# simonsysu/tfs

Measured on AMD Instinct MI355X. Metric: GiB/s CRC32 verify, device-resident 64 KiB files; 1/2/4/8 MI355X, higher is better.
Workload: dtype u8

## Files before the change

tfs_amd/csrc/crc_math.h:

```cpp
#pragma once
#include <cstdint>

namespace tfscrc {

constexpr uint32_t kPoly = 0xEDB88320u;

inline void make_byte_table(uint32_t t[256]) {
  for (uint32_t i = 0; i < 256; ++i) {
    uint32_t c = i;
    for (int k = 0; k < 8; ++k) c = (c & 1u) ? (c >> 1) ^ kPoly : (c >> 1);
    t[i] = c;
  }
}

inline void make_slice_tables(uint32_t s[][256], int nslices) {
  make_byte_table(s[0]);
  for (int k = 1; k < nslices; ++k)
    for (int b = 0; b < 256; ++b) s[k][b] = (s[k - 1][b] >> 8) ^ s[0][s[k - 1][b] & 0xffu];
}

inline uint32_t multmodp(uint32_t a, uint32_t b) {
  uint32_t m = 1u << 31, p = 0;
  for (;;) {
    if (a & m) {
      p ^= b;
      if ((a & (m - 1)) == 0) break;
    }
    m >>= 1;
    b = (b & 1u) ? (b >> 1) ^ kPoly : b >> 1;
  }
  return p;
}

inline uint32_t x2nmodp(uint64_t n, unsigned k) {
  uint32_t p = 1u << 31;
  uint32_t sq = 1u << 30;
  for (unsigned i = 0; i < k; ++i) sq = multmodp(sq, sq);
  while (n) {
    if (n & 1) p = multmodp(sq, p);
    n >>= 1;
    sq = multmodp(sq, sq);
  }
  return p;
}

inline uint32_t shift_bytes(uint32_t c, uint64_t nbytes) { return multmodp(x2nmodp(nbytes, 3), c); }

inline uint32_t shift_bytes_pow(uint32_t c, uint64_t nbytes) {
  struct Pow {
    uint32_t p[64];
    Pow() {
      p[0] = x2nmodp(1, 3);
      for (int k = 1; k < 64; ++k) p[k] = multmodp(p[k - 1], p[k - 1]);
    }
  };
  static const Pow pw;
  for (int k = 0; nbytes; ++k, nbytes >>= 1)
    if (nbytes & 1) c = multmodp(pw.p[k], c);
  return c;
}

inline void make_shift_table(uint32_t t[4][256], uint64_t nbytes) {
  const uint32_t k = x2nmodp(nbytes, 3);
  for (int j = 0; j < 4; ++j)
    for (uint32_t b = 0; b < 256; ++b) t[j][b] = multmodp(k, b << (8 * j));
}

inline void make_shift_table5(uint32_t t[7][32], uint64_t nbytes) {
  const uint32_t k = x2nmodp(nbytes, 3);
  for (int j = 0; j < 7; ++j)
    for (uint32_t e = 0; e < 32; ++e) t[j][e] = (j == 6 && e >= 4) ? 0u : multmodp(k, e << (5 * j));
}

}
```

tfs_amd/csrc/tfs_ec_abi.cpp:

```cpp
#include <hip/hip_runtime.h>

#include <cstdlib>
#include <cstring>
#include <mutex>
#include <vector>

#include "../../include/tfs_ec.h"
#include "crc_math.h"
#include "ec_math.h"

#include "ec_locate_plan.h"
#include "ec_marshal_plan.h"
#include "ec_read_plan.h"
#include "tfs_ec_device.h"

extern "C" int tfs_crc32_dev_malloc(tfs_crc_ctx* ctx, uint64_t bytes, void** d_ptr);
extern "C" int tfs_crc32_dev_free(tfs_crc_ctx* ctx, void* d_ptr);
extern "C" void* tfs_crc32_stream(tfs_crc_ctx* ctx);

using namespace tfsec;

namespace {
struct Plan {
  std::vector<int> sources, outputs;
// ... 172 lines not shown
int upload_read_tables(tfs_ec* ec) {
  void* d = nullptr;
  const int rc = tfs_crc32_dev_malloc(ec->ctx, sizeof(ReadTables), &d);
  if (rc) return rc;
  if (hipMemcpy(d, &read_tables(), sizeof(ReadTables), hipMemcpyHostToDevice) != hipSuccess) {
    tfs_crc32_dev_free(ec->ctx, d);
    return TFS_CRC_EXIT_DEVICE_ERROR;
  }
  ec->d_read_tab = static_cast<ReadTables*>(d);
  return TFS_SUCCESS;
}

int check_read(tfs_ec* ec, void* const* members, const int* sizes, int size, int target, int* row) {
  const Plan& p = ec->dec;
  if (!p.valid || !ec->d_read_tab) return TFS_EXIT_MATRIX_INVALID;
  if (size < 0 || size % kUnit != 0) return TFS_EXIT_SIZE_INVALID;
  if (target < 0 || target >= ec->dn) return TFS_EXIT_PARAMETER_ERROR;
  *row = -1;
  for (size_t o = 0; o < p.outputs.size(); ++o)
    if (p.outputs[o] == target) *row = int(o);
  if (*row < 0) return TFS_EXIT_PARAMETER_ERROR;
  if (!members) return TFS_EXIT_DATA_INVALID;
  for (int s : p.sources)
    if (!members[s] || (sizes && sizes[s] < size)) return TFS_EXIT_DATA_INVALID;
  return TFS_SUCCESS;
}

int launch_read(tfs_ec* ec, void* const* members, int size, int row, const void* d_jobs, uint32_t n, void* d_out,
                uint64_t out_cap, uint32_t* d_out_crc, int32_t* d_out_status, uint32_t* d_n_bad, hipStream_t st) {
  const Plan& p = ec->dec;
  const int S = int(p.sources.size());
  ReadArgs a;
  memset(&a, 0, sizeof a);
  for (int s = 0; s < S; ++s) a.src[s] = static_cast<const uint8_t*>(members[p.sources[s]]);
  a.masks = p.d_masks + size_t(row) * 8 * size_t(S) * 8;
  a.tab = ec->d_read_tab;
  a.jobs = static_cast<const ReadJob*>(d_jobs);
  a.out = static_cast<uint8_t*>(d_out);
  a.out_cap = out_cap;
  a.out_crc = d_out_crc;
  a.out_status = d_out_status;
  a.n_bad = d_n_bad;
  a.n = n;
  a.S = uint32_t(S);
  a.size = size;
  return launch_ec_read(a, st) == hipSuccess ? TFS_SUCCESS : TFS_CRC_EXIT_DEVICE_ERROR;
}


const MarshalTables& marshal_tables() {
  static const MarshalTables* t = [] {
    MarshalTables* r = new MarshalTables();
    tfscrc::make_slice_tables(r->slice, 4);
    tfscrc::make_shift_table(r->step_packet, kReadStepPacket);
    const uint32_t g = tfscrc::x2nmodp(8, 0), gi = tfscrc::x2nmodp(0xFFFFFFFFull - 8, 0);
    r->xpow[kMarshalPowBias] = 1u << 31;
    for (int i = kMarshalPowBias + 1; i < kMarshalPowN; ++i) r->xpow[i] = tfscrc::multmodp(g, r->xpow[i - 1]);
    for (int i = kMarshalPowBias - 1; i >= 0; --i) r->xpow[i] = tfscrc::multmodp(gi, r->xpow[i + 1]);
    return r;
  }();
  return *t;
}

int chunk_check(tfs_ec_marshal* m, int offset, int len, hipStream_t want, hipStream_t* st) {
  if (!m || !m->ec) return TFS_EXIT_PARAMETER_ERROR;
  if (want == hipStreamPerThread) return TFS_EXIT_PARAMETER_ERROR;
  *st = want ? want : static_cast<hipStream_t>(tfs_crc32_stream(m->ec->ctx));
  if (m->stream_set && *st != m->stream) return TFS_EXIT_PARAMETER_ERROR;
  if (offset != m->next || len <= 0 || offset % 4096 != 0 || len % kUnit != 0 || len > m->total - offset)
    return TFS_EXIT_PARAMETER_ERROR;
  if (len % 4096 != 0 && offset + len != m->total) return TFS_EXIT_PARAMETER_ERROR;
  return TFS_SUCCESS;
}

int marshal_check(tfs_ec_marshal* m, void* const* members, int offset, int len, hipStream_t want, hipStream_t* st) {
  const int rc = chunk_check(m, offset, len, want, st);
  if (rc) return rc;
  if (!members) return TFS_EXIT_DATA_INVALID;
  for (int i = 0; i < m->ec->dn + m->ec->pn; ++i)
    if (!members[i]) return TFS_EXIT_DATA_INVALID;
  return TFS_SUCCESS;
}

int marshal_launch(tfs_ec_marshal* m, void* const* members, int offset, int len, hipStream_t st) {
  tfs_ec* ec = m->ec;
  const Plan& p = ec->enc;
  if (m->plan.recs.empty()) return run_plan(ec, p, members, len, st);
  const int S = int(p.sources.size());
  for (size_t o0 = 0; o0 < p.outputs.size(); o0 += kMaxOutGroup) {
    const int og = int(std::min<size_t>(kMaxOutGroup, p.outputs.size() - o0));
    MarshalArgs a;
    memset(&a, 0, sizeof a);
    for (int s = 0; s < S; ++s) a.ec.src[s] = static_cast<const uint8_t*>(members[p.sources[s]]);
    for (int o = 0; o < og; ++o) a.ec.dst[o] = static_cast<uint8_t*>(members[p.outputs[o0 + o]]);
    a.ec.masks = p.d_masks + o0 * 8 * size_t(S) * 8;
    a.ec.S = uint32_t(S);
    a.ec.units = uint64_t(len) / kUnit;
    if (o0) {
      if (launch_ec_apply(a.ec, og, 0, st) != hipSuccess) return TFS_CRC_EXIT_DEVICE_ERROR;
      continue;
    }
    a.tab = ec->d_marshal_tab;
    a.recs = m->d_recs;
    a.first = m->d_first;
    a.cont = m->d_cont;
    a.tail = m->d_tail;
    a.hdr = m->d_hdr;
// ... 891 lines not shown
```

tfs_amd/csrc/tfs_ec_device.h:

```cpp
#pragma once
#include <hip/hip_runtime.h>
#include <stdint.h>

#include "ec_update_plan.h"

namespace tfsec {

constexpr int kMaxMembersDev = 12;
constexpr int kMaxOutGroup = 4;

struct EcArgs {
  const uint8_t* src[kMaxMembersDev];
  uint8_t* dst[kMaxOutGroup];
  const uint32_t* masks;
  uint32_t S;
  uint64_t units;
};

hipError_t launch_ec_apply(const EcArgs& a, int og, int variant, hipStream_t stream);

struct ReadJob {
  uint64_t file_id;
  uint64_t out_offset;
  int32_t offset, size;
  uint32_t flags, reserved;
};
static_assert(sizeof(ReadJob) == 32, "read job layout");
constexpr uint32_t kReadRange = 1u;
constexpr int kReadWaves = 8;
constexpr unsigned kReadMaxGrid = 4096;
constexpr uint32_t kReadStepPacket = 128, kReadStepTile = 4096u * kReadWaves - 896u;
constexpr int kReadPowBias = 4095;
constexpr int kReadPowN = kReadPowBias + 4096 * (kReadWaves - 1) + 3192 + 1;
struct ReadTables {
  uint32_t slice[4][256];
  uint32_t step_packet[4][256];
  uint32_t step_tile[4][256];
  uint32_t xpow[kReadPowN];
};
#ifdef __HIP__
__attribute__((host)) __attribute__((device))
#endif
inline int32_t read_job_check(const ReadJob& jb, int32_t member_size, uint64_t out_cap, uint32_t* A, uint32_t* E) {
  const int64_t cover_end = (int64_t(jb.offset) + int64_t(jb.size) + 1023) & ~int64_t(1023);
  if (jb.offset < 0 || jb.size < 0 || cover_end > int64_t(member_size)) return -1016;
  *A = uint32_t(jb.offset) & ~1023u;
  *E = uint32_t(cover_end);
  if ((jb.out_offset & 1023u) != 0u || jb.out_offset > out_cap || uint64_t(*E - *A) > out_cap - jb.out_offset)
    return -1016;
  if (!(jb.flags & kReadRange) && jb.size <= 36) return -8034;
  return 0;
}

struct ReadArgs {
  const uint8_t* src[kMaxMembersDev];
  const uint32_t* masks;
  const ReadTables* tab;
  const ReadJob* jobs;
  uint8_t* out;
  uint64_t out_cap;
  uint32_t* out_crc;
  int32_t* out_status;
  uint32_t* n_bad;
  uint32_t n, S;
  int32_t size;
};

hipError_t launch_ec_read(const ReadArgs& a, hipStream_t stream);

struct MarshalRec {
  uint32_t H, P1;
  uint32_t id_lo, id_hi;
};
constexpr int kMarshalPowBias = 4095;
constexpr int kMarshalPowN = kMarshalPowBias + 4096 + 1;
constexpr uint32_t kMarshalHdrWords = 9;
struct MarshalTables {
  uint32_t slice[4][256];
  uint32_t step_packet[4][256];
  uint32_t xpow[kMarshalPowN];
};
struct MarshalArgs {
  EcArgs ec;
  const MarshalTables* tab;
  const MarshalRec* recs;
  const uint32_t* first;
  uint32_t* cont;
  uint32_t* tail;
  uint32_t* hdr;
  uint32_t mend[kMaxMembersDev];
  uint32_t tile0;
  uint32_t ntiles;
};
hipError_t launch_ec_marshal(const MarshalArgs& a, int og, hipStream_t stream);

struct MarshalFoldArgs {
  const MarshalTables* tab;
  const MarshalRec* recs;
  const uint32_t* rec_member;
  const uint32_t* cont;
  const uint32_t* tail;
  const uint32_t* hdr;
  const uint32_t* pow_tile;
  uint32_t* out_crc;
  int32_t* out_status;
  uint32_t n, ntiles;
};
hipError_t launch_ec_marshal_fold(const MarshalFoldArgs& a, hipStream_t stream);

constexpr uint32_t kReinstateNoSlot = 0xFFFFFFFFu;
struct ReinstateArgs {
  MarshalArgs m;
  uint32_t src_slot[kMaxMembersDev];
  uint32_t out_slot[kMaxOutGroup];
};
hipError_t launch_ec_reinstate(const ReinstateArgs& a, int og, hipStream_t stream);

struct ScrubArgs {
  MarshalArgs m;
  const uint8_t* par[kMaxOutGroup];
  uint32_t* pbad;
  uint32_t o0;
};
hipError_t launch_ec_scrub(const ScrubArgs& a, int og, bool walk, hipStream_t stream);

struct ScrubCountArgs {
  const uint32_t* pbad;
  uint32_t* units;
  uint8_t* map;
  uint32_t ntiles;
};
hipError_t launch_ec_scrub_count(const ScrubCountArgs& a, int pn, hipStream_t stream);

struct LocateResult {
// ... 32 lines not shown
```

tfs_amd/csrc/tfs_ec_kernels.hip:

```cpp
#include <hip/hip_runtime.h>
#include <stdint.h>

#include "tfs_crc_device.h"
#include "tfs_ec_device.h"

namespace tfsec {

typedef unsigned int u32x2 __attribute__((ext_vector_type(2)));
typedef const __attribute__((address_space(1))) u32x2* gu64p;
typedef __attribute__((address_space(1))) u32x2* gu64wp;

__device__ __forceinline__ u32x2 ld64nt(const uint8_t* p) {
  return __builtin_nontemporal_load(reinterpret_cast<gu64p>(reinterpret_cast<uintptr_t>(p)));
}
__device__ __forceinline__ void st64nt(uint8_t* p, u32x2 v) {
  __builtin_nontemporal_store(v, reinterpret_cast<gu64wp>(reinterpret_cast<uintptr_t>(p)));
}
__device__ __forceinline__ uint32_t xand(uint32_t acc, uint32_t in, uint32_t m) {
  return __builtin_amdgcn_bitop3_b32(acc, in, m, 0x78);
}

template <int OG>
__device__ __forceinline__ void ec_apply_body(const EcArgs& a, const uint32_t* __restrict__ masks) {
  const int lane = threadIdx.x & 63;
// ... 344 lines not shown
        const int64_t sk = int64_t(P0) - int64_t(q), ek = int64_t(P1) - int64_t(q);
        if (sk > 0 || ek < 8) {
          const uint64_t mk = ek <= sk ? 0ull : rd_low_bytes(ek) & ~rd_low_bytes(sk);
          lo &= uint32_t(mk);
          hi &= uint32_t(mk >> 32);
        }
        const uint32_t piece = rd_slice4(sl, rd_slice4(sl, lo) ^ hi);
        crc = rd_lut4(c == 0 ? stt : stp, crc) ^ piece;
      }
    }
    if (range) {
      if (threadIdx.x == 0) {
        a.out_crc[j] = 0u;
        a.out_status[j] = tfscrc::kSuccess;
      }
      continue;
    }
    {
      const uint32_t tl = nt - 1u - ((nt - 1u - wv) & (kReadWaves - 1u));
      const int32_t dl = wv < nt ? int32_t(4096u * (nt - 1u - tl)) + 3192 - int32_t(1024u * u + off) : 0;
      const int32_t pad = int32_t(A + 4096u * nt - P1);
      crc = rd_multmodp(a.tab->xpow[kReadPowBias + dl - pad], crc);
#pragma unroll
      for (int m = 32; m >= 1; m >>= 1) crc ^= __shfl_xor(crc, m, 64);
      if (lane == 0) part[wv] = crc;
    }
    __syncthreads();
    if (threadIdx.x == 0) {
      uint32_t v = 0;
#pragma unroll
      for (int w = 0; w < kReadWaves; ++w) v ^= part[w];
      const uint64_t id = uint64_t(hdr[0]) | (uint64_t(hdr[1]) << 32);
      const int32_t fsize = int32_t(hdr[3]);
      const uint32_t fcrc = hdr[8];
      if (id != jb.file_id) status = tfscrc::kExitFileInfoError;
      else if (fsize != jb.size) status = tfscrc::kExitSyncFileError;
      else if (fcrc != v) status = tfscrc::kExitCheckCrcError;
      a.out_crc[j] = v;
      a.out_status[j] = status;
      if (status != tfscrc::kSuccess) ++bad;
    }
    __syncthreads();
  }
  if (threadIdx.x == 0 && bad && a.n_bad) atomicAdd(a.n_bad, bad);
}

hipError_t launch_ec_read(const ReadArgs& a, hipStream_t stream) {
  if (a.n == 0) return hipSuccess;
  const uint32_t blocks = a.n < kReadMaxGrid ? a.n : kReadMaxGrid;
  hipLaunchKernelGGL(ec_read_kernel, dim3(blocks), dim3(64 * kReadWaves), 0, stream, a);
  return hipGetLastError();
}

template <int OG>
__global__ void __launch_bounds__(256, OG <= 3 ? 4 : 3)
    ec_marshal_kernel(MarshalArgs a, const uint32_t* __restrict__ masks, const MarshalTables* __restrict__ tab,
                      const MarshalRec* __restrict__ recs, const uint32_t* __restrict__ first) {
  __shared__ uint32_t lt[2 * 1024];
  const uint32_t* sl = lt;
  const uint32_t* stp = lt + 1024;
  const int lane = threadIdx.x & 63;
  const uint32_t u = uint32_t(lane) >> 4;
  const uint32_t off = 8u * uint32_t(lane & 15);
  const uint32_t S = a.ec.S;
  const uint64_t ntl = (a.ec.units + 3) / 4;
  const uint64_t t = uint64_t(blockIdx.x) * 4u + __builtin_amdgcn_readfirstlane(threadIdx.x >> 6);
  const uint64_t unit = t * 4 + u;
  const bool ok = t < ntl && unit < a.ec.units;
  const uint64_t base = unit * 1024u + off;
  u32x2 in[8];
#pragma unroll
  for (int c = 0; c < 8; ++c) in[c] = ok ? ld64nt(a.ec.src[0] + base + 128u * c) : u32x2{0u, 0u};
  {
    const uint32_t* g = reinterpret_cast<const uint32_t*>(tab);
    for (uint32_t i = threadIdx.x; i < 2u * 1024u; i += 256u) lt[i] = g[i];
  }
  __syncthreads();
  if (t >= ntl) return;
  const uint32_t T = a.tile0 + uint32_t(t);
  const uint32_t tile_lo = T << 12, tile_hi = tile_lo + 4096u;
  const uint32_t q0 = tile_lo + 1024u * u + off;
  const int32_t dl = 3192 - int32_t(1024u * u + off);
  uint8_t* const hdr8 = reinterpret_cast<uint8_t*>(a.hdr);
  u32x2 acc[OG][8];
#pragma unroll
  for (int o = 0; o < OG; ++o)
#pragma unroll
    for (int r = 0; r < 8; ++r) acc[o][r] = u32x2{0u, 0u};
  for (uint32_t s = 0; s < S; ++s) {
    u32x2 nx[8];
    const bool more = s + 1 < S;
    const uint8_t* np = a.ec.src[more ? s + 1 : s];
#pragma unroll
    for (int c = 0; c < 8; ++c) nx[c] = (ok && more) ? ld64nt(np + base + 128u * c) : u32x2{0u, 0u};
#pragma unroll
    for (int o = 0; o < OG; ++o)
#pragma unroll
      for (int r = 0; r < 8; ++r) {
        const uint32_t* m = masks + ((uint32_t(o) * 8u + uint32_t(r)) * S + s) * 8u;
#pragma unroll
        for (int c = 0; c < 8; ++c) {
          const uint32_t mk = m[c];
          acc[o][r].x = xand(acc[o][r].x, in[c].x, mk);
          acc[o][r].y = xand(acc[o][r].y, in[c].y, mk);
        }
      }
    const uint32_t rend = a.mend[s];
    for (uint32_t r = __builtin_amdgcn_readfirstlane(first[size_t(s) * a.ntiles + T]); r < rend; ++r) {
      const uint32_t H = __builtin_amdgcn_readfirstlane(recs[r].H);
      const uint32_t P1 = __builtin_amdgcn_readfirstlane(recs[r].P1);
      if (H >= tile_hi) break;
      const uint32_t P0 = H + uint32_t(tfscrc::kFileInfoSize);
      const uint32_t live = 0u - uint32_t(P1 > tile_lo);
      if (P0 > tile_lo) {
#pragma unroll
        for (int c = 0; c < 8; ++c) {
          const uint32_t q = q0 + 128u * c;
          if (q + 8u > H && q < P0) {
            const uint64_t v = uint64_t(in[c].x & live) | (uint64_t(in[c].y & live) << 32);
#pragma unroll
            for (int b = 0; b < 8; ++b) {
              const uint32_t p = q + uint32_t(b) - H;
              if (p < uint32_t(tfscrc::kFileInfoSize)) hdr8[size_t(r) * (4u * kMarshalHdrWords) + p] = uint8_t(v >> (8 * b));
            }
          }
        }
      }
      if (P0 >= tile_hi) continue;
      uint32_t crc = 0;
      if (P0 <= tile_lo && P1 >= tile_hi) {
#pragma unroll
        for (int c = 0; c < 8; ++c) {
          const uint32_t piece = rd_slice4(sl, rd_slice4(sl, in[c].x & live) ^ (in[c].y & live));
          crc = c == 0 ? piece : rd_lut4(stp, crc) ^ piece;
        }
      } else {
#pragma unroll
        for (int c = 0; c < 8; ++c) {
          const uint32_t q = q0 + 128u * c;
          uint32_t lo = in[c].x & live, hi = in[c].y & live;
          const int64_t sk = int64_t(P0) - int64_t(q), ek = int64_t(P1) - int64_t(q);
          if (sk > 0 || ek < 8) {
            const uint64_t mk = ek <= sk ? 0ull : rd_low_bytes(ek) & ~rd_low_bytes(sk);
            lo &= uint32_t(mk);
            hi &= uint32_t(mk >> 32);
          }
          const uint32_t piece = rd_slice4(sl, rd_slice4(sl, lo) ^ hi);
          crc = c == 0 ? piece : rd_lut4(stp, crc) ^ piece;
        }
      }
      const bool on = P1 > tile_hi;
      const int32_t pad = P1 >= tile_hi ? 0 : int32_t(tile_hi - P1);
      crc = rd_multmodp(tab->xpow[kMarshalPowBias + dl - pad], crc);
#pragma unroll
      for (int m = 32; m >= 1; m >>= 1) crc ^= __shfl_xor(crc, m, 64);
      if (lane == 0) {
        if (on) a.cont[size_t(s) * a.ntiles + T] = crc;
        else a.tail[r] = crc;
      }
    }
#pragma unroll
    for (int c = 0; c < 8; ++c) in[c] = nx[c];
  }
  if (ok) {
#pragma unroll
    for (int o = 0; o < OG; ++o)
#pragma unroll
      for (int r = 0; r < 8; ++r) st64nt(a.ec.dst[o] + base + 128u * r, acc[o][r]);
  }
}

hipError_t launch_ec_marshal(const MarshalArgs& a, int og, hipStream_t stream) {
  if (a.ec.units == 0) return hipSuccess;
  const uint64_t ntl = (a.ec.units + 3) / 4;
  const dim3 g(static_cast<unsigned>((ntl + 3) / 4)), b(256);
  switch (og) {
    case 1: hipLaunchKernelGGL(ec_marshal_kernel<1>, g, b, 0, stream, a, a.ec.masks, a.tab, a.recs, a.first); break;
    case 2: hipLaunchKernelGGL(ec_marshal_kernel<2>, g, b, 0, stream, a, a.ec.masks, a.tab, a.recs, a.first); break;
    case 3: hipLaunchKernelGGL(ec_marshal_kernel<3>, g, b, 0, stream, a, a.ec.masks, a.tab, a.recs, a.first); break;
    default: hipLaunchKernelGGL(ec_marshal_kernel<4>, g, b, 0, stream, a, a.ec.masks, a.tab, a.recs, a.first); break;
  }
  return hipGetLastError();
}

__global__ void __launch_bounds__(256) ec_marshal_fold_kernel(MarshalFoldArgs a) {
  const uint32_t lane = threadIdx.x & 63u;
  const uint32_t r = blockIdx.x * 4u + __builtin_amdgcn_readfirstlane(threadIdx.x >> 6);
  if (r >= a.n) return;
  const MarshalRec rc = a.recs[r];
  const uint32_t P0 = rc.H + uint32_t(tfscrc::kFileInfoSize), P1 = rc.P1;
  const uint32_t t0 = P0 >> 12, tl = (P1 - 1u) >> 12;
  const uint32_t nc = tl - t0;
  uint32_t c = 0;
  if (nc) {
    const uint32_t* cont = a.cont + size_t(a.rec_member[r]) * a.ntiles;
    const uint32_t R = (nc + 63u) / 64u;
    const uint32_t b = min(t0 + lane * R, tl), e = min(b + R, tl);
    const uint32_t x4k = a.pow_tile[1];
    for (uint32_t t = b; t < e; ++t) c = rd_multmodp(x4k, c) ^ cont[t];
    c = rd_multmodp(a.pow_tile[tl - e], c);
#pragma unroll
    for (int m = 32; m >= 1; m >>= 1) c ^= __shfl_xor(c, m, 64);
  }
  if (lane == 0) {
    const uint32_t v = rd_multmodp(a.tab->xpow[kMarshalPowBias + int32_t(P1 - (tl << 12))], c) ^ a.tail[r];
    const uint32_t* h = a.hdr + size_t(r) * kMarshalHdrWords;
    const int32_t size = int32_t(P1 - rc.H);
    int32_t status = tfscrc::kSuccess;
    if (h[0] != rc.id_lo || h[1] != rc.id_hi) status = tfscrc::kExitFileInfoError;
    else if (int32_t(h[3]) != size) status = tfscrc::kExitSyncFileError;
    else if (h[8] != v) status = tfscrc::kExitCheckCrcError;
    a.out_crc[r] = v;
    a.out_status[r] = status;
  }
}

hipError_t launch_ec_marshal_fold(const MarshalFoldArgs& a, hipStream_t stream) {
  if (a.n == 0) return hipSuccess;
  hipLaunchKernelGGL(ec_marshal_fold_kernel, dim3((a.n + 3u) / 4u), dim3(256), 0, stream, a);
  return hipGetLastError();
}

struct ReinstateWalk {
  const uint32_t* sl;
  const uint32_t* stp;
  uint32_t T, tile_lo, tile_hi, q0, ntiles;
  int32_t dl;
  int lane;
};

template <bool QREC = false>
__device__ __forceinline__ void reinstate_walk(const u32x2 (&pc)[8], const ReinstateWalk& w, uint32_t slot, uint32_t rend,
                                               const MarshalTables* __restrict__ tab, const MarshalRec* __restrict__ recs,
                                               const uint32_t* __restrict__ first, uint32_t* cont, uint32_t* tail,
                                               uint8_t* hdr8) {
  const uint32_t tile_lo = w.tile_lo, tile_hi = w.tile_hi;
  for (uint32_t r = __builtin_amdgcn_readfirstlane(first[size_t(slot) * w.ntiles + w.T]); r < rend; ++r) {
    const uint32_t H = __builtin_amdgcn_readfirstlane(recs[r].H);
    const uint32_t P1 = __builtin_amdgcn_readfirstlane(recs[r].P1);
    if (H >= tile_hi) break;
    const uint32_t P0 = H + uint32_t(tfscrc::kFileInfoSize);
    const uint32_t live = 0u - uint32_t(P1 > tile_lo);
    const uint32_t q0 = QREC ? w.q0 + ~live : w.q0;
    if (P0 > tile_lo) {
#pragma unroll
      for (int c = 0; c < 8; ++c) {
        const uint32_t q = q0 + 128u * c;
        if (q + 8u > H && q < P0) {
          const uint64_t v = uint64_t(pc[c].x & live) | (uint64_t(pc[c].y & live) << 32);
#pragma unroll
          for (int b = 0; b < 8; ++b) {
            const uint32_t p = q + uint32_t(b) - H;
            if (p < uint32_t(tfscrc::kFileInfoSize)) hdr8[size_t(r) * (4u * kMarshalHdrWords) + p] = uint8_t(v >> (8 * b));
          }
        }
      }
    }
    if (P0 >= tile_hi) continue;
    uint32_t crc = 0;
    if (P0 <= tile_lo && P1 >= tile_hi) {
#pragma unroll
      for (int c = 0; c < 8; ++c) {
        const uint32_t piece = rd_slice4(w.sl, rd_slice4(w.sl, pc[c].x & live) ^ (pc[c].y & live));
        crc = c == 0 ? piece : rd_lut4(w.stp, crc) ^ piece;
      }
    } else {
#pragma unroll
      for (int c = 0; c < 8; ++c) {
        const uint32_t q = q0 + 128u * c;
        uint32_t lo = pc[c].x & live, hi = pc[c].y & live;
        const int64_t sk = int64_t(P0) - int64_t(q), ek = int64_t(P1) - int64_t(q);
        if (sk > 0 || ek < 8) {
          const uint64_t mk = ek <= sk ? 0ull : rd_low_bytes(ek) & ~rd_low_bytes(sk);
          lo &= uint32_t(mk);
          hi &= uint32_t(mk >> 32);
        }
        const uint32_t piece = rd_slice4(w.sl, rd_slice4(w.sl, lo) ^ hi);
        crc = c == 0 ? piece : rd_lut4(w.stp, crc) ^ piece;
      }
    }
    const bool on = P1 > tile_hi;
    const int32_t pad = P1 >= tile_hi ? 0 : int32_t(tile_hi - P1);
    crc = rd_multmodp(tab->xpow[kMarshalPowBias + w.dl - pad], crc);
#pragma unroll
    for (int m = 32; m >= 1; m >>= 1) crc ^= __shfl_xor(crc, m, 64);
    if (w.lane == 0) {
      if (on) cont[size_t(slot) * w.ntiles + w.T] = crc;
      else tail[r] = crc;
    }
  }
}

template <int OG>
__global__ void __launch_bounds__(256, OG <= 2 ? 4 : 3)
    ec_reinstate_kernel(ReinstateArgs a, const uint32_t* __restrict__ masks, const MarshalTables* __restrict__ tab,
                        const MarshalRec* __restrict__ recs, const uint32_t* __restrict__ first) {
  __shared__ uint32_t lt[2 * 1024];
  const int lane = threadIdx.x & 63;
  const uint32_t u = uint32_t(lane) >> 4;
  const uint32_t off = 8u * uint32_t(lane & 15);
  const uint32_t S = a.m.ec.S;
  const uint64_t ntl = (a.m.ec.units + 3) / 4;
  const uint64_t t = uint64_t(blockIdx.x) * 4u + __builtin_amdgcn_readfirstlane(threadIdx.x >> 6);
  const uint64_t unit = t * 4 + u;
  const bool ok = t < ntl && unit < a.m.ec.units;
  const uint64_t base = unit * 1024u + off;
  u32x2 in[8];
#pragma unroll
  for (int c = 0; c < 8; ++c) in[c] = ok ? ld64nt(a.m.ec.src[0] + base + 128u * c) : u32x2{0u, 0u};
  {
    const uint32_t* g = reinterpret_cast<const uint32_t*>(tab);
    for (uint32_t i = threadIdx.x; i < 2u * 1024u; i += 256u) lt[i] = g[i];
  }
  __syncthreads();
  if (t >= ntl) return;
  ReinstateWalk w;
  w.sl = lt;
  w.stp = lt + 1024;
  w.T = a.m.tile0 + uint32_t(t);
  w.tile_lo = w.T << 12;
  w.tile_hi = w.tile_lo + 4096u;
  w.q0 = w.tile_lo + 1024u * u + off;
  w.ntiles = a.m.ntiles;
  w.dl = 3192 - int32_t(1024u * u + off);
  w.lane = lane;
  uint8_t* const hdr8 = reinterpret_cast<uint8_t*>(a.m.hdr);
  u32x2 acc[OG][8];
#pragma unroll
  for (int o = 0; o < OG; ++o)
#pragma unroll
    for (int r = 0; r < 8; ++r) acc[o][r] = u32x2{0u, 0u};
  for (uint32_t s = 0; s < S; ++s) {
    u32x2 nx[8];
    const bool more = s + 1 < S;
    const uint8_t* np = a.m.ec.src[more ? s + 1 : s];
#pragma unroll
    for (int c = 0; c < 8; ++c) nx[c] = (ok && more) ? ld64nt(np + base + 128u * c) : u32x2{0u, 0u};
#pragma unroll
    for (int o = 0; o < OG; ++o)
#pragma unroll
      for (int r = 0; r < 8; ++r) {
        const uint32_t* m = masks + ((uint32_t(o) * 8u + uint32_t(r)) * S + s) * 8u;
#pragma unroll
        for (int c = 0; c < 8; ++c) {
          const uint32_t mk = m[c];
          acc[o][r].x = xand(acc[o][r].x, in[c].x, mk);
          acc[o][r].y = xand(acc[o][r].y, in[c].y, mk);
        }
      }
    const uint32_t slot = a.src_slot[s];
    if (slot != kReinstateNoSlot) reinstate_walk(in, w, slot, a.m.mend[slot], tab, recs, first, a.m.cont, a.m.tail, hdr8);
#pragma unroll
    for (int c = 0; c < 8; ++c) in[c] = nx[c];
  }
  if (ok) {
#pragma unroll
    for (int o = 0; o < OG; ++o)
#pragma unroll
      for (int r = 0; r < 8; ++r) st64nt(a.m.ec.dst[o] + base + 128u * r, acc[o][r]);
  }
#pragma unroll
  for (int o = 0; o < OG; ++o) {
    const uint32_t slot = a.out_slot[o];
    if (slot != kReinstateNoSlot) reinstate_walk(acc[o], w, slot, a.m.mend[slot], tab, recs, first, a.m.cont, a.m.tail, hdr8);
  }
}

hipError_t launch_ec_reinstate(const ReinstateArgs& a, int og, hipStream_t stream) {
  if (a.m.ec.units == 0) return hipSuccess;
  const uint64_t ntl = (a.m.ec.units + 3) / 4;
  const dim3 g(static_cast<unsigned>((ntl + 3) / 4)), b(256);
  switch (og) {
    case 1: hipLaunchKernelGGL(ec_reinstate_kernel<1>, g, b, 0, stream, a, a.m.ec.masks, a.m.tab, a.m.recs, a.m.first); break;
    case 2: hipLaunchKernelGGL(ec_reinstate_kernel<2>, g, b, 0, stream, a, a.m.ec.masks, a.m.tab, a.m.recs, a.m.first); break;
    case 3: hipLaunchKernelGGL(ec_reinstate_kernel<3>, g, b, 0, stream, a, a.m.ec.masks, a.m.tab, a.m.recs, a.m.first); break;
    default: hipLaunchKernelGGL(ec_reinstate_kernel<4>, g, b, 0, stream, a, a.m.ec.masks, a.m.tab, a.m.recs, a.m.first); break;
  }
  return hipGetLastError();
}

__device__ __forceinline__ u32x2 ld64nt_at(const uint8_t* p, uint32_t o) {
  typedef const __attribute__((address_space(1))) uint8_t* g8p;
  return __builtin_nontemporal_load(reinterpret_cast<gu64p>(reinterpret_cast<g8p>(reinterpret_cast<uintptr_t>(p)) + o));
}

template <int OG, bool WALK>
__global__ void __launch_bounds__(256, OG <= 3 ? 4 : 3)
    ec_scrub_kernel(ScrubArgs a, const uint32_t* __restrict__ masks, const MarshalTables* __restrict__ tab,
                    const MarshalRec* __restrict__ recs, const uint32_t* __restrict__ first) {
  __shared__ uint32_t lt[WALK ? 2 * 1024 : 1];
  const int lane = threadIdx.x & 63;
  const uint32_t u = uint32_t(lane) >> 4;
  const uint32_t off = 8u * uint32_t(lane & 15);
  const uint32_t S = a.m.ec.S;
  __builtin_assume(S != 0u);
  const uint64_t ntl = (a.m.ec.units + 3) / 4;
  const uint64_t t = uint64_t(blockIdx.x) * 4u + __builtin_amdgcn_readfirstlane(threadIdx.x >> 6);
  const uint64_t unit = t * 4 + u;
  const bool ok = t < ntl && unit < a.m.ec.units;
  const uint32_t base = uint32_t(unit) * 1024u + off;
  u32x2 in[8];
#pragma unroll
  for (int c = 0; c < 8; ++c) in[c] = ok ? ld64nt_at(a.m.ec.src[0], base + 128u * c) : u32x2{0u, 0u};
  if (WALK) {
    const uint32_t* g = reinterpret_cast<const uint32_t*>(tab);
    for (uint32_t i = threadIdx.x; i < 2u * 1024u; i += 256u) lt[i] = g[i];
    __syncthreads();
  }
  if (t >= ntl) return;
  const uint32_t T = a.m.tile0 + uint32_t(t);
  ReinstateWalk w;
  w.sl = lt;
  w.stp = lt + (WALK ? 1024 : 0);
  w.T = T;
  w.tile_lo = T << 12;
  w.tile_hi = w.tile_lo + 4096u;
  w.q0 = w.tile_lo + 1024u * u + off;
  w.ntiles = a.m.ntiles;
  w.dl = 3192 - int32_t(1024u * u + off);
  w.lane = lane;
  uint8_t* const hdr8 = reinterpret_cast<uint8_t*>(a.m.hdr);
  u32x2 acc[OG][8];
#pragma unroll
  for (int o = 0; o < OG; ++o)
#pragma unroll
    for (int r = 0; r < 8; ++r) acc[o][r] = u32x2{0u, 0u};
  for (uint32_t s = 0; s < S; ++s) {
    u32x2 nx[8];
    const uint8_t* np = s + 1 < S ? a.m.ec.src[s + 1] : a.par[0];
#pragma unroll
    for (int c = 0; c < 8; ++c) nx[c] = ok ? ld64nt_at(np, base + 128u * c) : u32x2{0u, 0u};
#pragma unroll
    for (int o = 0; o < OG; ++o)
#pragma unroll
      for (int r = 0; r < 8; ++r) {
        const uint32_t* m = masks + ((uint32_t(o) * 8u + uint32_t(r)) * S + s) * 8u;
#pragma unroll
        for (int c = 0; c < 8; ++c) {
          const uint32_t mk = m[c];
          acc[o][r].x = xand(acc[o][r].x, in[c].x, mk);
          acc[o][r].y = xand(acc[o][r].y, in[c].y, mk);
        }
      }
    if (WALK) reinstate_walk<true>(in, w, s, a.m.mend[s], tab, recs, first, a.m.cont, a.m.tail, hdr8);
#pragma unroll
    for (int c = 0; c < 8; ++c) in[c] = nx[c];
  }
#pragma unroll
  for (int o = 0; o < OG; ++o) {
    u32x2 nx[8];
#pragma unroll
    for (int c = 0; c < 8; ++c) nx[c] = (ok && o + 1 < OG) ? ld64nt_at(a.par[o + 1 < OG ? o + 1 : o], base + 128u * c) : u32x2{0u, 0u};
    uint32_t d = 0;
#pragma unroll
    for (int r = 0; r < 8; ++r) d |= (acc[o][r].x ^ in[r].x) | (acc[o][r].y ^ in[r].y);
    const uint64_t b = __builtin_amdgcn_ballot_w64(d != 0u);
    const uint32_t bits = uint32_t((b & 0xFFFFull) != 0ull) | (uint32_t(((b >> 16) & 0xFFFFull) != 0ull) << 1) |
                          (uint32_t(((b >> 32) & 0xFFFFull) != 0ull) << 2) | (uint32_t((b >> 48) != 0ull) << 3);
    if (__builtin_amdgcn_mbcnt_hi(~0u, __builtin_amdgcn_mbcnt_lo(~0u, 0u)) == 0u) a.pbad[size_t(a.o0 + uint32_t(o)) * a.m.ntiles + T] = bits;
#pragma unroll
    for (int c = 0; c < 8; ++c) in[c] = nx[c];
  }
}

template <bool WALK>
static void launch_scrub_og(const ScrubArgs& a, int og, dim3 g, dim3 b, hipStream_t stream) {
  switch (og) {
    case 1: hipLaunchKernelGGL((ec_scrub_kernel<1, WALK>), g, b, 0, stream, a, a.m.ec.masks, a.m.tab, a.m.recs, a.m.first); break;
    case 2: hipLaunchKernelGGL((ec_scrub_kernel<2, WALK>), g, b, 0, stream, a, a.m.ec.masks, a.m.tab, a.m.recs, a.m.first); break;
    case 3: hipLaunchKernelGGL((ec_scrub_kernel<3, WALK>), g, b, 0, stream, a, a.m.ec.masks, a.m.tab, a.m.recs, a.m.first); break;
    default: hipLaunchKernelGGL((ec_scrub_kernel<4, WALK>), g, b, 0, stream, a, a.m.ec.masks, a.m.tab, a.m.recs, a.m.first); break;
  }
}

hipError_t launch_ec_scrub(const ScrubArgs& a, int og, bool walk, hipStream_t stream) {
  if (a.m.ec.units == 0) return hipSuccess;
  const uint64_t ntl = (a.m.ec.units + 3) / 4;
  const dim3 g(static_cast<unsigned>((ntl + 3) / 4)), b(256);
  if (walk) launch_scrub_og<true>(a, og, g, b, stream);
  else launch_scrub_og<false>(a, og, g, b, stream);
  return hipGetLastError();
}

__global__ void __launch_bounds__(1024) ec_scrub_count_kernel(ScrubCountArgs a) {
  __shared__ uint32_t part[16];
  const uint32_t p = blockIdx.x;
  const uint32_t* w = a.pbad + size_t(p) * a.ntiles;
  uint8_t* mp = a.map + size_t(p) * a.ntiles;
  uint32_t c = 0;
  for (uint32_t T0 = threadIdx.x; T0 < a.ntiles; T0 += 4096u) {
    uint32_t v[4];
#pragma unroll
    for (int k = 0; k < 4; ++k) v[k] = T0 + 1024u * k < a.ntiles ? w[T0 + 1024u * k] & 15u : 0u;
#pragma unroll
    for (int k = 0; k < 4; ++k)
      if (T0 + 1024u * k < a.ntiles) {
        mp[T0 + 1024u * k] = uint8_t(v[k]);
// ... 256 lines not shown
```

Before: 6276.

## Replace per-record CRC shift/xor-reduce with DPP tree combine and gap-advanced slice tables

The per-wave CRC combine in the marshal, reinstate and scrub record walks is reworked. Each lane's 8-byte pieces are now folded with a precomputed slice table that already includes the 120-byte gap, so the per-chunk step_packet lookup goes away. The global xpow multmodp plus 6-step shuffle reduction is replaced by a 6-level DPP row-shift tree using 5-bit shift tables staged in LDS. Tail padding is moved into the fold kernel, and the record walk now runs before the EC xor-and loop. This trades extra LDS footprint (about 1.3K more words per block) and table lookups for fewer cross-lane shuffles and global reads per record.

Result: slower. 6135 (-2.2%).

```diff
diff --git a/tfs_amd/csrc/crc_math.h b/tfs_amd/csrc/crc_math.h
--- a/tfs_amd/csrc/crc_math.h
+++ b/tfs_amd/csrc/crc_math.h
@@ -66,6 +66,12 @@
     for (uint32_t b = 0; b < 256; ++b) t[j][b] = multmodp(k, b << (8 * j));
 }
 
+inline void make_slice_tables_advanced(uint32_t a[4][256], const uint32_t s[4][256], uint64_t nbytes) {
+  const uint32_t k = x2nmodp(nbytes, 3);
+  for (int j = 0; j < 4; ++j)
+    for (int b = 0; b < 256; ++b) a[j][b] = multmodp(k, s[j][b]);
+}
+
 inline void make_shift_table5(uint32_t t[7][32], uint64_t nbytes) {
   const uint32_t k = x2nmodp(nbytes, 3);
   for (int j = 0; j < 7; ++j)
diff --git a/tfs_amd/csrc/tfs_ec_abi.cpp b/tfs_amd/csrc/tfs_ec_abi.cpp
--- a/tfs_amd/csrc/tfs_ec_abi.cpp
+++ b/tfs_amd/csrc/tfs_ec_abi.cpp
@@ -248,7 +248,8 @@
   static const MarshalTables* t = [] {
     MarshalTables* r = new MarshalTables();
     tfscrc::make_slice_tables(r->slice, 4);
-    tfscrc::make_shift_table(r->step_packet, kReadStepPacket);
+    tfscrc::make_slice_tables_advanced(r->slice_gap, r->slice, kMarshalPieceGap);
+    for (int j = 0; j < kMarshalTreeLevels; ++j) tfscrc::make_shift_table5(r->tree[j], kMarshalTreeBytes[j]);
     const uint32_t g = tfscrc::x2nmodp(8, 0), gi = tfscrc::x2nmodp(0xFFFFFFFFull - 8, 0);
     r->xpow[kMarshalPowBias] = 1u << 31;
     for (int i = kMarshalPowBias + 1; i < kMarshalPowN; ++i) r->xpow[i] = tfscrc::multmodp(g, r->xpow[i - 1]);
diff --git a/tfs_amd/csrc/tfs_ec_device.h b/tfs_amd/csrc/tfs_ec_device.h
--- a/tfs_amd/csrc/tfs_ec_device.h
+++ b/tfs_amd/csrc/tfs_ec_device.h
@@ -75,11 +75,17 @@
 constexpr int kMarshalPowBias = 4095;
 constexpr int kMarshalPowN = kMarshalPowBias + 4096 + 1;
 constexpr uint32_t kMarshalHdrWords = 9;
+constexpr uint32_t kMarshalPieceGap = 120;
+constexpr int kMarshalTreeLevels = 6;
+constexpr uint32_t kMarshalTreeBytes[kMarshalTreeLevels] = {8, 16, 32, 64, 1024, 2048};
 struct MarshalTables {
   uint32_t slice[4][256];
-  uint32_t step_packet[4][256];
+  uint32_t slice_gap[4][256];
+  uint32_t tree[kMarshalTreeLevels][7][32];
   uint32_t xpow[kMarshalPowN];
 };
+constexpr uint32_t kMarshalLdsWords = 2u * 1024u + kMarshalTreeLevels * 224u;
+static_assert(sizeof(MarshalTables) == 4u * (kMarshalLdsWords + kMarshalPowN), "the staged tables lie in front, without gaps");
 struct MarshalArgs {
   EcArgs ec;
   const MarshalTables* tab;
diff --git a/tfs_amd/csrc/tfs_ec_kernels.hip b/tfs_amd/csrc/tfs_ec_kernels.hip
--- a/tfs_amd/csrc/tfs_ec_kernels.hip
+++ b/tfs_amd/csrc/tfs_ec_kernels.hip
@@ -420,13 +420,97 @@
   return hipGetLastError();
 }
 
+struct RecordWalk {
+  const uint32_t* lt;
+  uint32_t T, tile_lo, tile_hi, q0, ntiles;
+};
+
+__device__ __forceinline__ uint32_t walk_piece(const uint32_t* sl, const uint32_t* second, uint32_t c, uint32_t lo, uint32_t hi) {
+  return rd_slice4(second, rd_slice4(sl, c ^ lo) ^ hi);
+}
+__device__ __forceinline__ uint32_t walk_shift5(const uint32_t* t, uint32_t c) {
+  return t[c & 31u] ^ t[32u + ((c >> 5) & 31u)] ^ t[64u + ((c >> 10) & 31u)] ^ t[96u + ((c >> 15) & 31u)] ^
+         t[128u + ((c >> 20) & 31u)] ^ t[160u + ((c >> 25) & 31u)] ^ t[192u + (c >> 30)];
+}
+template <int CTRL>
+__device__ __forceinline__ uint32_t walk_level(const uint32_t* t, uint32_t c) {
+  const uint32_t lower = uint32_t(__builtin_amdgcn_update_dpp(0, int(c), CTRL, 0xF, 0xF, true));
+  return walk_shift5(t, lower) ^ c;
+}
+__device__ __forceinline__ uint32_t walk_combine(const uint32_t* tree, uint32_t c) {
+  c = walk_level<0x111>(tree, c);
+  c = walk_level<0x112>(tree + 224, c);
+  c = walk_level<0x114>(tree + 448, c);
+  c = walk_level<0x118>(tree + 672, c);
+  c = walk_level<0x142>(tree + 896, c);
+  return walk_level<0x143>(tree + 1120, c);
+}
+
+template <bool QREC = false>
+__device__ __forceinline__ void record_walk(const u32x2 (&pc)[8], const RecordWalk& w, uint32_t slot, uint32_t rend,
+                                            const MarshalRec* __restrict__ recs, const uint32_t* __restrict__ first,
+                                            uint32_t* cont, uint32_t* tail, uint8_t* hdr8) {
+  const uint32_t tile_lo = w.tile_lo, tile_hi = w.tile_hi;
+  const uint32_t* const sl = w.lt;
+  const uint32_t* const sg = w.lt + 1024;
+  for (uint32_t r = __builtin_amdgcn_readfirstlane(first[size_t(slot) * w.ntiles + w.T]); r < rend; ++r) {
+    const uint32_t H = __builtin_amdgcn_readfirstlane(recs[r].H);
+    const uint32_t P1 = __builtin_amdgcn_readfirstlane(recs[r].P1);
+    if (H >= tile_hi) break;
+    const uint32_t P0 = H + uint32_t(tfscrc::kFileInfoSize);
+    const uint32_t live = 0u - uint32_t(P1 > tile_lo);
+    const uint32_t q0 = QREC ? w.q0 + ~live : w.q0;
+    if (P0 > tile_lo) {
+#pragma unroll
+      for (int c = 0; c < 8; ++c) {
+        const uint32_t q = q0 + 128u * c;
+        if (q + 8u > H && q < P0) {
+          const uint64_t v = uint64_t(pc[c].x & live) | (uint64_t(pc[c].y & live) << 32);
+#pragma unroll
+          for (int b = 0; b < 8; ++b) {
+            const uint32_t p = q + uint32_t(b) - H;
+            if (p < uint32_t(tfscrc::kFileInfoSize)) hdr8[size_t(r) * (4u * kMarshalHdrWords) + p] = uint8_t(v >> (8 * b));
+          }
+        }
+      }
+    }
+    if (P0 >= tile_hi) continue;
+    uint32_t crc = 0;
+    if (P0 <= tile_lo && P1 >= tile_hi) {
+#pragma unroll
+      for (int c = 0; c < 8; ++c) crc = walk_piece(sl, c == 7 ? sl : sg, crc, pc[c].x & live, pc[c].y & live);
+    } else {
+#pragma unroll
+      for (int c = 0; c < 8; ++c) {
+        const uint32_t q = q0 + 128u * c;
+        uint32_t lo = pc[c].x & live, hi = pc[c].y & live;
+        const int64_t sk = int64_t(P0) - int64_t(q), ek = int64_t(P1) - int64_t(q);
+        if (sk > 0 || ek < 8) {
+          const uint64_t mk = ek <= sk ? 0ull : rd_low_bytes(ek) & ~rd_low_bytes(sk);
+          lo &= uint32_t(mk);
+          hi &= uint32_t(mk >> 32);
+        }
+        crc = walk_piece(sl, c == 7 ? sl : sg, crc, lo, hi);
+      }
+    }
+    crc = walk_combine(w.lt + 2048, crc);
+    if (__builtin_amdgcn_mbcnt_hi(~0u, __builtin_amdgcn_mbcnt_lo(~0u, 0u)) == 63u) {
+      if (P1 > tile_hi) cont[size_t(slot) * w.ntiles + w.T] = crc;
+      else tail[r] = crc;
+    }
+  }
+}
+
+__device__ __forceinline__ void stage_walk_tables(uint32_t* lt, const MarshalTables* tab) {
+  const uint32_t* g = reinterpret_cast<const uint32_t*>(tab);
+  for (uint32_t i = threadIdx.x; i < kMarshalLdsWords; i += 256u) lt[i] = g[i];
+}
+
 template <int OG>
 __global__ void __launch_bounds__(256, OG <= 3 ? 4 : 3)
     ec_marshal_kernel(MarshalArgs a, const uint32_t* __restrict__ masks, const MarshalTables* __restrict__ tab,
                       const MarshalRec* __restrict__ recs, const uint32_t* __restrict__ first) {
-  __shared__ uint32_t lt[2 * 1024];
-  const uint32_t* sl = lt;
-  const uint32_t* stp = lt + 1024;
+  __shared__ uint32_t lt[kMarshalLdsWords];
   const int lane = threadIdx.x & 63;
   const uint32_t u = uint32_t(lane) >> 4;
   const uint32_t off = 8u * uint32_t(lane & 15);
@@ -439,16 +523,16 @@
   u32x2 in[8];
 #pragma unroll
   for (int c = 0; c < 8; ++c) in[c] = ok ? ld64nt(a.ec.src[0] + base + 128u * c) : u32x2{0u, 0u};
-  {
-    const uint32_t* g = reinterpret_cast<const uint32_t*>(tab);
-    for (uint32_t i = threadIdx.x; i < 2u * 1024u; i += 256u) lt[i] = g[i];
-  }
+  stage_walk_tables(lt, tab);
   __syncthreads();
   if (t >= ntl) return;
-  const uint32_t T = a.tile0 + uint32_t(t);
-  const uint32_t tile_lo = T << 12, tile_hi = tile_lo + 4096u;
-  const uint32_t q0 = tile_lo + 1024u * u + off;
-  const int32_t dl = 3192 - int32_t(1024u * u + off);
+  RecordWalk w;
+  w.lt = lt;
+  w.T = a.tile0 + uint32_t(t);
+  w.tile_lo = w.T << 12;
+  w.tile_hi = w.tile_lo + 4096u;
+  w.q0 = w.tile_lo + 1024u * u + off;
+  w.ntiles = a.ntiles;
   uint8_t* const hdr8 = reinterpret_cast<uint8_t*>(a.hdr);
   u32x2 acc[OG][8];
 #pragma unroll
@@ -461,6 +545,7 @@
     const uint8_t* np = a.ec.src[more ? s + 1 : s];
 #pragma unroll
     for (int c = 0; c < 8; ++c) nx[c] = (ok && more) ? ld64nt(np + base + 128u * c) : u32x2{0u, 0u};
+    record_walk(in, w, s, a.mend[s], recs, first, a.cont, a.tail, hdr8);
 #pragma unroll
     for (int o = 0; o < OG; ++o)
 #pragma unroll
@@ -473,60 +558,6 @@
           acc[o][r].y = xand(acc[o][r].y, in[c].y, mk);
         }
       }
-    const uint32_t rend = a.mend[s];
-    for (uint32_t r = __builtin_amdgcn_readfirstlane(first[size_t(s) * a.ntiles + T]); r < rend; ++r) {
-      const uint32_t H = __builtin_amdgcn_readfirstlane(recs[r].H);
-      const uint32_t P1 = __builtin_amdgcn_readfirstlane(recs[r].P1);
-      if (H >= tile_hi) break;
-      const uint32_t P0 = H + uint32_t(tfscrc::kFileInfoSize);
-      const uint32_t live = 0u - uint32_t(P1 > tile_lo);
-      if (P0 > tile_lo) {
-#pragma unroll
-        for (int c = 0; c < 8; ++c) {
-          const uint32_t q = q0 + 128u * c;
-          if (q + 8u > H && q < P0) {
-            const uint64_t v = uint64_t(in[c].x & live) | (uint64_t(in[c].y & live) << 32);
-#pragma unroll
-            for (int b = 0; b < 8; ++b) {
-              const uint32_t p = q + uint32_t(b) - H;
-              if (p < uint32_t(tfscrc::kFileInfoSize)) hdr8[size_t(r) * (4u * kMarshalHdrWords) + p] = uint8_t(v >> (8 * b));
-            }
-          }
-        }
-      }
-      if (P0 >= tile_hi) continue;
-      uint32_t crc = 0;
-      if (P0 <= tile_lo && P1 >= tile_hi) {
-#pragma unroll
-        for (int c = 0; c < 8; ++c) {
-          const uint32_t piece = rd_slice4(sl, rd_slice4(sl, in[c].x & live) ^ (in[c].y & live));
-          crc = c == 0 ? piece : rd_lut4(stp, crc) ^ piece;
-        }
-      } else {
-#pragma unroll
-        for (int c = 0; c < 8; ++c) {
-          const uint32_t q = q0 + 128u * c;
-          uint32_t lo = in[c].x & live, hi = in[c].y & live;
-          const int64_t sk = int64_t(P0) - int64_t(q), ek = int64_t(P1) - int64_t(q);
-          if (sk > 0 || ek < 8) {
-            const uint64_t mk = ek <= sk ? 0ull : rd_low_bytes(ek) & ~rd_low_bytes(sk);
-            lo &= uint32_t(mk);
-            hi &= uint32_t(mk >> 32);
-          }
-          const uint32_t piece = rd_slice4(sl, rd_slice4(sl, lo) ^ hi);
-          crc = c == 0 ? piece : rd_lut4(stp, crc) ^ piece;
-        }
-      }
-      const bool on = P1 > tile_hi;
-      const int32_t pad = P1 >= tile_hi ? 0 : int32_t(tile_hi - P1);
-      crc = rd_multmodp(tab->xpow[kMarshalPowBias + dl - pad], crc);
-#pragma unroll
-      for (int m = 32; m >= 1; m >>= 1) crc ^= __shfl_xor(crc, m, 64);
-      if (lane == 0) {
-        if (on) a.cont[size_t(s) * a.ntiles + T] = crc;
-        else a.tail[r] = crc;
-      }
-    }
 #pragma unroll
     for (int c = 0; c < 8; ++c) in[c] = nx[c];
   }
@@ -556,6 +587,7 @@
   const uint32_t r = blockIdx.x * 4u + __builtin_amdgcn_readfirstlane(threadIdx.x >> 6);
   if (r >= a.n) return;
   const MarshalRec rc = a.recs[r];
+  const uint32_t tail = a.tail[r];
   const uint32_t P0 = rc.H + uint32_t(tfscrc::kFileInfoSize), P1 = rc.P1;
   const uint32_t t0 = P0 >> 12, tl = (P1 - 1u) >> 12;
   const uint32_t nc = tl - t0;
@@ -570,8 +602,12 @@
 #pragma unroll
     for (int m = 32; m >= 1; m >>= 1) c ^= __shfl_xor(c, m, 64);
   }
+  const int32_t pad = int32_t(((tl + 1u) << 12) - P1);
+  const bool second = lane == 1u;
+  const uint32_t unpad = a.tab->xpow[kMarshalPowBias - pad], on = a.tab->xpow[kMarshalPowBias + 4096 - pad];
+  uint32_t v = rd_multmodp(second ? unpad : on, second ? tail : c);
+  v ^= uint32_t(__builtin_amdgcn_readlane(int(v), 1));
   if (lane == 0) {
-    const uint32_t v = rd_multmodp(a.tab->xpow[kMarshalPowBias + int32_t(P1 - (tl << 12))], c) ^ a.tail[r];
     const uint32_t* h = a.hdr + size_t(r) * kMarshalHdrWords;
     const int32_t size = int32_t(P1 - rc.H);
     int32_t status = tfscrc::kSuccess;
@@ -589,81 +625,11 @@
   return hipGetLastError();
 }
 
-struct ReinstateWalk {
-  const uint32_t* sl;
-  const uint32_t* stp;
-  uint32_t T, tile_lo, tile_hi, q0, ntiles;
-  int32_t dl;
-  int lane;
-};
-
-template <bool QREC = false>
-__device__ __forceinline__ void reinstate_walk(const u32x2 (&pc)[8], const ReinstateWalk& w, uint32_t slot, uint32_t rend,
-                                               const MarshalTables* __restrict__ tab, const MarshalRec* __restrict__ recs,
-                                               const uint32_t* __restrict__ first, uint32_t* cont, uint32_t* tail,
-                                               uint8_t* hdr8) {
-  const uint32_t tile_lo = w.tile_lo, tile_hi = w.tile_hi;
-  for (uint32_t r = __builtin_amdgcn_readfirstlane(first[size_t(slot) * w.ntiles + w.T]); r < rend; ++r) {
-    const uint32_t H = __builtin_amdgcn_readfirstlane(recs[r].H);
-    const uint32_t P1 = __builtin_amdgcn_readfirstlane(recs[r].P1);
-    if (H >= tile_hi) break;
-    const uint32_t P0 = H + uint32_t(tfscrc::kFileInfoSize);
-    const uint32_t live = 0u - uint32_t(P1 > tile_lo);
-    const uint32_t q0 = QREC ? w.q0 + ~live : w.q0;
-    if (P0 > tile_lo) {
-#pragma unroll
-      for (int c = 0; c < 8; ++c) {
-        const uint32_t q = q0 + 128u * c;
-        if (q + 8u > H && q < P0) {
-          const uint64_t v = uint64_t(pc[c].x & live) | (uint64_t(pc[c].y & live) << 32);
-#pragma unroll
-          for (int b = 0; b < 8; ++b) {
-            const uint32_t p = q + uint32_t(b) - H;
-            if (p < uint32_t(tfscrc::kFileInfoSize)) hdr8[size_t(r) * (4u * kMarshalHdrWords) + p] = uint8_t(v >> (8 * b));
-          }
-        }
-      }
-    }
-    if (P0 >= tile_hi) continue;
-    uint32_t crc = 0;
-    if (P0 <= tile_lo && P1 >= tile_hi) {
-#pragma unroll
-      for (int c = 0; c < 8; ++c) {
-        const uint32_t piece = rd_slice4(w.sl, rd_slice4(w.sl, pc[c].x & live) ^ (pc[c].y & live));
-        crc = c == 0 ? piece : rd_lut4(w.stp, crc) ^ piece;
-      }
-    } else {
-#pragma unroll
-      for (int c = 0; c < 8; ++c) {
-        const uint32_t q = q0 + 128u * c;
-        uint32_t lo = pc[c].x & live, hi = pc[c].y & live;
-        const int64_t sk = int64_t(P0) - int64_t(q), ek = int64_t(P1) - int64_t(q);
-        if (sk > 0 || ek < 8) {
-          const uint64_t mk = ek <= sk ? 0ull : rd_low_bytes(ek) & ~rd_low_bytes(sk);
-          lo &= uint32_t(mk);
-          hi &= uint32_t(mk >> 32);
-        }
-        const uint32_t piece = rd_slice4(w.sl, rd_slice4(w.sl, lo) ^ hi);
-        crc = c == 0 ? piece : rd_lut4(w.stp, crc) ^ piece;
-      }
-    }
-    const bool on = P1 > tile_hi;
-    const int32_t pad = P1 >= tile_hi ? 0 : int32_t(tile_hi - P1);
-    crc = rd_multmodp(tab->xpow[kMarshalPowBias + w.dl - pad], crc);
-#pragma unroll
-    for (int m = 32; m >= 1; m >>= 1) crc ^= __shfl_xor(crc, m, 64);
-    if (w.lane == 0) {
-      if (on) cont[size_t(slot) * w.ntiles + w.T] = crc;
-      else tail[r] = crc;
-    }
-  }
-}
-
 template <int OG>
 __global__ void __launch_bounds__(256, OG <= 2 ? 4 : 3)
     ec_reinstate_kernel(ReinstateArgs a, const uint32_t* __restrict__ masks, const MarshalTables* __restrict__ tab,
                         const MarshalRec* __restrict__ recs, const uint32_t* __restrict__ first) {
-  __shared__ uint32_t lt[2 * 1024];
+  __shared__ uint32_t lt[kMarshalLdsWords];
   const int lane = threadIdx.x & 63;
   const uint32_t u = uint32_t(lane) >> 4;
   const uint32_t off = 8u * uint32_t(lane & 15);
@@ -676,22 +642,16 @@
   u32x2 in[8];
 #pragma unroll
   for (int c = 0; c < 8; ++c) in[c] = ok ? ld64nt(a.m.ec.src[0] + base + 128u * c) : u32x2{0u, 0u};
-  {
-    const uint32_t* g = reinterpret_cast<const uint32_t*>(tab);
-    for (uint32_t i = threadIdx.x; i < 2u * 1024u; i += 256u) lt[i] = g[i];
-  }
+  stage_walk_tables(lt, tab);
   __syncthreads();
   if (t >= ntl) return;
-  ReinstateWalk w;
-  w.sl = lt;
-  w.stp = lt + 1024;
+  RecordWalk w;
+  w.lt = lt;
   w.T = a.m.tile0 + uint32_t(t);
   w.tile_lo = w.T << 12;
   w.tile_hi = w.tile_lo + 4096u;
   w.q0 = w.tile_lo + 1024u * u + off;
   w.ntiles = a.m.ntiles;
-  w.dl = 3192 - int32_t(1024u * u + off);
-  w.lane = lane;
   uint8_t* const hdr8 = reinterpret_cast<uint8_t*>(a.m.hdr);
   u32x2 acc[OG][8];
 #pragma unroll
@@ -704,6 +664,8 @@
     const uint8_t* np = a.m.ec.src[more ? s + 1 : s];
 #pragma unroll
     for (int c = 0; c < 8; ++c) nx[c] = (ok && more) ? ld64nt(np + base + 128u * c) : u32x2{0u, 0u};
+    const uint32_t slot = a.src_slot[s];
+    if (slot != kReinstateNoSlot) record_walk(in, w, slot, a.m.mend[slot], recs, first, a.m.cont, a.m.tail, hdr8);
 #pragma unroll
     for (int o = 0; o < OG; ++o)
 #pragma unroll
@@ -716,8 +678,6 @@
           acc[o][r].y = xand(acc[o][r].y, in[c].y, mk);
         }
       }
-    const uint32_t slot = a.src_slot[s];
-    if (slot != kReinstateNoSlot) reinstate_walk(in, w, slot, a.m.mend[slot], tab, recs, first, a.m.cont, a.m.tail, hdr8);
 #pragma unroll
     for (int c = 0; c < 8; ++c) in[c] = nx[c];
   }
@@ -730,7 +690,7 @@
 #pragma unroll
   for (int o = 0; o < OG; ++o) {
     const uint32_t slot = a.out_slot[o];
-    if (slot != kReinstateNoSlot) reinstate_walk(acc[o], w, slot, a.m.mend[slot], tab, recs, first, a.m.cont, a.m.tail, hdr8);
+    if (slot != kReinstateNoSlot) record_walk(acc[o], w, slot, a.m.mend[slot], recs, first, a.m.cont, a.m.tail, hdr8);
   }
 }
 
@@ -756,7 +716,7 @@
 __global__ void __launch_bounds__(256, OG <= 3 ? 4 : 3)
     ec_scrub_kernel(ScrubArgs a, const uint32_t* __restrict__ masks, const MarshalTables* __restrict__ tab,
                     const MarshalRec* __restrict__ recs, const uint32_t* __restrict__ first) {
-  __shared__ uint32_t lt[WALK ? 2 * 1024 : 1];
+  __shared__ uint32_t lt[WALK ? kMarshalLdsWords : 1];
   const int lane = threadIdx.x & 63;
   const uint32_t u = uint32_t(lane) >> 4;
   const uint32_t off = 8u * uint32_t(lane & 15);
@@ -771,22 +731,18 @@
 #pragma unroll
   for (int c = 0; c < 8; ++c) in[c] = ok ? ld64nt_at(a.m.ec.src[0], base + 128u * c) : u32x2{0u, 0u};
   if (WALK) {
-    const uint32_t* g = reinterpret_cast<const uint32_t*>(tab);
-    for (uint32_t i = threadIdx.x; i < 2u * 1024u; i += 256u) lt[i] = g[i];
+    stage_walk_tables(lt, tab);
     __syncthreads();
   }
   if (t >= ntl) return;
   const uint32_t T = a.m.tile0 + uint32_t(t);
-  ReinstateWalk w;
-  w.sl = lt;
-  w.stp = lt + (WALK ? 1024 : 0);
+  RecordWalk w;
+  w.lt = lt;
   w.T = T;
   w.tile_lo = T << 12;
   w.tile_hi = w.tile_lo + 4096u;
   w.q0 = w.tile_lo + 1024u * u + off;
   w.ntiles = a.m.ntiles;
-  w.dl = 3192 - int32_t(1024u * u + off);
-  w.lane = lane;
   uint8_t* const hdr8 = reinterpret_cast<uint8_t*>(a.m.hdr);
   u32x2 acc[OG][8];
 #pragma unroll
@@ -798,6 +754,7 @@
     const uint8_t* np = s + 1 < S ? a.m.ec.src[s + 1] : a.par[0];
 #pragma unroll
     for (int c = 0; c < 8; ++c) nx[c] = ok ? ld64nt_at(np, base + 128u * c) : u32x2{0u, 0u};
+    if (WALK) record_walk<true>(in, w, s, a.m.mend[s], recs, first, a.m.cont, a.m.tail, hdr8);
 #pragma unroll
     for (int o = 0; o < OG; ++o)
 #pragma unroll
@@ -810,7 +767,6 @@
           acc[o][r].y = xand(acc[o][r].y, in[c].y, mk);
         }
       }
-    if (WALK) reinstate_walk<true>(in, w, s, a.m.mend[s], tab, recs, first, a.m.cont, a.m.tail, hdr8);
 #pragma unroll
     for (int c = 0; c < 8; ++c) in[c] = nx[c];
   }
```
